# TheCacophonyProject/classifier-pipeline

Hardware: AMD Instinct MI355X
Metric: CPTV frames/s end-to-end (track+classify) at 160x120 (higher is better)
Workload: dtype u16/i32 track stage (f32 normalise, f64 gates); f32 crop/tile; f32 CNN (stride-1 3x3 convs of stages 2-4 (+ the stride-2 one): two fp16 planes per operand rounded to nearest (11 + 11 significand bits), power-of-two range scaling, 3 fp16 MFMAs per K step, device-side rerun in the exact split if an ac

## Files before the change

classifier-pipeline_amd/csrc/cpx_api.cpp:

```cpp
#include <hip/hip_runtime.h>

#include <algorithm>
#include <cmath>
#include <cstdio>
#include <cstdlib>
#include <cstring>
#include <new>
#include <string>
#include <vector>

#include "cpx_internal.h"

static_assert(sizeof(cpx_component) == 32, "cpx_component layout is part of the ABI");
static_assert(sizeof(cpx_frame_info) == 80, "cpx_frame_info layout is part of the ABI");
static_assert(sizeof(cpx_frame_meta) == 24, "cpx_frame_meta layout is part of the ABI");
static_assert(sizeof(cpx_config) == 48, "cpx_config layout is part of the ABI");
static_assert(sizeof(cpx_region_ref) == 24 && sizeof(cpx_track_limits) == 32 && sizeof(cpx_crop_req) == 32,
              "classification request layouts are part of the ABI");
static_assert(sizeof(cpx_filter_params) == 72 && sizeof(cpx_track_summary) == 120,
              "end-of-clip layouts are part of the ABI");
static_assert(sizeof(cpx_region) == 56, "cpx_region layout is part of the ABI");
static_assert(sizeof(cpx_track_record) == 32, "cpx_track_record layout is part of the ABI");
static_assert(sizeof(cpx_track_params) == 120, "cpx_track_params layout is part of the ABI");

namespace {

struct WsLayout {
  size_t bg, wsum, kcnt, filt, cstate, u8, carry, bgavg, big, total;
};

WsLayout ws_layout(const cpx_config& c, int B, bool need_filt_state) {
  const size_t P = (size_t)c.width * c.height;
  WsLayout l{};
  size_t off = 0;
  l.bg = off;
  off = align_up(off + (size_t)B * 2 * P * sizeof(uint16_t), 256);
  l.wsum = off;
  off = align_up(off + (size_t)B * P * sizeof(uint32_t), 256);
  l.kcnt = off;
  off = align_up(off + (size_t)B * P * sizeof(uint16_t), 256);
  l.filt = off;
  if (need_filt_state) off = align_up(off + (size_t)B * 2 * P * sizeof(float), 256);
  l.cstate = off;
  off = align_up(off + (size_t)B * sizeof(cpx::ClipState), 256);
  l.u8 = off;
  off = align_up(off + (size_t)B * 2 * P, 256);
  l.carry = off;
  off = align_up(off + (size_t)B * 2 * sizeof(cpx::FrameCarry), 256);
  l.bgavg = off;
  off = align_up(off + (size_t)B * sizeof(double), 256);
  l.big = off;
  if (c.max_components > cpx::track_lds_components())
    off = align_up(off + (size_t)B * 9 * c.max_components * sizeof(uint32_t), 256);
  l.total = off;
  return l;
}

struct Schedule {
  std::vector<int> clip_first, proc_off, proc_idx, proc_ffc, order;
  int total = 0, max_proc = 0;
};

int build_schedule(cpx_handle* h, const int32_t* clip_offsets, const cpx_frame_meta* meta, int B, Schedule* sc) {
  sc->total = clip_offsets[B];
  sc->clip_first.resize(B);
  sc->proc_off.assign(B + 1, 0);
  sc->proc_idx.reserve(sc->total);
  sc->proc_ffc.reserve(sc->total);
  for (int b = 0; b < B; ++b) {
    const int f0 = clip_offsets[b], f1 = clip_offsets[b + 1];
    if (f1 <= f0) return fail(h, CPX_ERR_INVALID, "empty clip in batch");
    sc->clip_first[b] = f0;
    for (int f = f0; f < f1; ++f) {
      if (meta[f].background_frame) continue;
      sc->proc_idx.push_back(f);
      int ffc = 0;
      if (meta[f].has_times) ffc = (meta[f].time_on_ms - meta[f].last_ffc_ms) < 9 ? 1 : 0;
      sc->proc_ffc.push_back(ffc);
    }
    sc->proc_off[b + 1] = (int)sc->proc_idx.size();
    const int np = sc->proc_off[b + 1] - sc->proc_off[b];
    if (np > h->cfg.max_frames) return fail(h, CPX_ERR_INVALID, "clip longer than max_frames");
    sc->max_proc = std::max(sc->max_proc, np);
  }
  sc->order.resize(B);
  for (int b = 0; b < B; ++b) sc->order[b] = b;
  std::stable_sort(sc->order.begin(), sc->order.end(), [&](int x, int y) {
    return sc->proc_off[x + 1] - sc->proc_off[x] > sc->proc_off[y + 1] - sc->proc_off[y];
  });
  return CPX_OK;
}

int upload_schedule(cpx_handle* h, const Schedule& sc, int B) {
  const int n = std::max((int)sc.proc_idx.size(), 1);
  const size_t ints = (size_t)B + (B + 1) + 2 * (size_t)n + (size_t)B;
  if (ints > h->sched_ints) {
    if (h->sched_dev) hipFree(h->sched_dev);
    h->sched_dev = nullptr;
    h->sched_ints = 0;
    hipError_t e = hipMalloc((void**)&h->sched_dev, ints * sizeof(int));
    if (e != hipSuccess) return fail(h, CPX_ERR_NOMEM, "schedule hipMalloc", e);
    h->sched_ints = ints;
  }
  std::vector<int> flat(ints, 0);
  std::copy(sc.clip_first.begin(), sc.clip_first.end(), flat.begin());
  std::copy(sc.proc_off.begin(), sc.proc_off.end(), flat.begin() + B);
  std::copy(sc.proc_idx.begin(), sc.proc_idx.end(), flat.begin() + B + (B + 1));
  std::copy(sc.proc_ffc.begin(), sc.proc_ffc.end(), flat.begin() + B + (B + 1) + n);
  std::copy(sc.order.begin(), sc.order.end(), flat.begin() + B + (B + 1) + 2 * (size_t)n);
  CPX_HIP(h, hipMemcpyAsync(h->sched_dev, flat.data(), ints * sizeof(int), hipMemcpyHostToDevice, h->stream));
  CPX_HIP(h, hipStreamSynchronize(h->stream));
  return CPX_OK;
}

}

extern "C" {

int cpx_abi_version(void) { return CPX_ABI_VERSION; }

int cpx_create(int device_id, const cpx_config* cfg, cpx_handle** out) {
  if (!cfg || !out) return CPX_ERR_INVALID;
  *out = nullptr;
  int ndev = 0;
  if (hipGetDeviceCount(&ndev) != hipSuccess || ndev <= 0) return CPX_ERR_NO_DEVICE;
  if (device_id < 0 || device_id >= ndev) return CPX_ERR_INVALID;
  const int W = cfg->width, H = cfg->height;
  if (W <= 0 || H <= 0 || (W % 8) != 0 || W >= 192 || W * H > cpx::track_max_pixels() || H < 5 || W < 8)
    return CPX_ERR_UNSUPPORTED;
  if (cfg->edge_pixels < 0 || 2 * cfg->edge_pixels >= std::min(W, H) || cfg->window < 1 ||
      cfg->max_components < 1 || cfg->max_frames < 1 || cfg->max_frames > 65534)
    return CPX_ERR_INVALID;
  cpx_handle* h = new (std::nothrow) cpx_handle();
  if (!h) return CPX_ERR_NOMEM;
  h->device = device_id;
  h->cfg = *cfg;
  if (hipSetDevice(device_id) != hipSuccess || hipStreamCreateWithFlags(&h->stream, hipStreamNonBlocking) != hipSuccess ||
      hipStreamCreateWithFlags(&h->stream2, hipStreamNonBlocking) != hipSuccess ||
      hipEventCreateWithFlags(&h->ev_median, hipEventDisableTiming) != hipSuccess ||
      hipEventCreate(&h->ev0) != hipSuccess || hipEventCreate(&h->ev1) != hipSuccess) {
    cpx_destroy(h);
    return CPX_ERR_HIP;
  }
  h->wtab_len = 65536;
  h->wtab_host.resize(h->wtab_len);
  std::vector<double>& wt = h->wtab_host;
  double w = 0.0;
  for (int k = 0; k < h->wtab_len; ++k) {
    wt[k] = w;
    w = w + cfg->weight_add;
  }
  if (cfg->denoise) {
    if (!cpx::nlm_supported(W, H)) {
      cpx_destroy(h);
      return CPX_ERR_UNSUPPORTED;
    }
    const int fixed_point_mult = (int)(2147483647LL / (21 * 21 * 255));
    std::vector<int> lut(64, 0);
    for (int a2 = 0; a2 < 64; ++a2) {
      const double wv = std::exp(-((double)a2 * (64.0 / 49.0)) / 9.0);
      const double wr = std::nearbyint((double)fixed_point_mult * wv);
      lut[a2] = (wr < 0.001 * fixed_point_mult) ? 0 : (int)wr;
    }
    if (lut[63] != 0 || hipMalloc((void**)&h->nlm_lut_dev, 64 * sizeof(int)) != hipSuccess ||
// ... 3 lines not shown
    }
  }
  std::vector<uint32_t> thr(h->wtab_len);
  for (int k = 0; k < h->wtab_len; ++k) {
    const double wk = wt[k], m = std::nearbyint(wk);
    const bool exact = (wk == m), near = !exact && std::fabs(wk - m) < 1e-6;
    double hi = near ? m + 1.0 : std::floor(wk) + 1.0;
    if (!(hi >= 0.0)) hi = 0.0;
    if (hi > 536870912.0) hi = 536870912.0;
    thr[k] = 2u * (uint32_t)hi - (near ? 1u : 0u);
  }
  if (hipMalloc((void**)&h->wthr_dev, thr.size() * sizeof(uint32_t)) != hipSuccess ||
      hipMemcpy(h->wthr_dev, thr.data(), thr.size() * sizeof(uint32_t), hipMemcpyHostToDevice) != hipSuccess) {
    cpx_destroy(h);
    return CPX_ERR_HIP;
  }
  if (hipMalloc(&h->wtab_dev, wt.size() * sizeof(double)) != hipSuccess ||
      hipMemcpy(h->wtab_dev, wt.data(), wt.size() * sizeof(double), hipMemcpyHostToDevice) != hipSuccess ||
      cpx::frame_kernel_attr_setup() != 0) {
    cpx_destroy(h);
    return CPX_ERR_HIP;
  }
  if (const char* env = std::getenv("CPX_TRACK_PACKED_STATE")) h->packed_state_ok = std::atoi(env) != 0;
  if (const char* env = std::getenv("CPX_CNN_FUSE_CONV1")) h->fuse_conv1 = std::atoi(env) != 0;
  if (const char* env = std::getenv("CPX_TRACK_PER_STEP")) h->track_per_step = std::atoi(env) != 0;
  if (const char* env = std::getenv("CPX_CNN_FUSE_SHORTCUT")) h->fuse_shortcut = std::atoi(env) != 0;
  if (const char* env = std::getenv("CPX_CNN_BLOCK_FUSION")) h->block_fusion = std::min(std::max(std::atoi(env), 0), 2);
  if (const char* env = std::getenv("CPX_CNN_MATH")) {
    if (!std::strcmp(env, "f32")) h->cnn_math = CPX_CNN_MATH_F32;
    else if (!std::strcmp(env, "bf16x3")) h->cnn_math = CPX_CNN_MATH_BF16X3;
    else if (!std::strcmp(env, "bf16x2")) h->cnn_math = CPX_CNN_MATH_BF16X2;
    else if (!std::strcmp(env, "fp16x2")) h->cnn_math = CPX_CNN_MATH_FP16X2;
  }
  *out = h;
  return CPX_OK;
}

void cpx_destroy(cpx_handle* h) {
  if (!h) return;
  hipSetDevice(h->device);
  if (h->stream) hipStreamSynchronize(h->stream);
  for (cpx_cnn* c : h->cnns) cnn_free(c);
  h->cnns.clear();
  for (cpx_mog2* m : h->mog2s) mog2_free(m);
  h->mog2s.clear();
  for (cpx_graph* g : h->graphs) graph_free(g);
  h->graphs.clear();
  if (h->graph_arena) hipFree(h->graph_arena);
  if (h->ws) hipFree(h->ws);
  if (h->wtab_dev) hipFree(h->wtab_dev);
  if (h->wthr_dev) hipFree(h->wthr_dev);
  if (h->nlm_lut_dev) hipFree(h->nlm_lut_dev);
  if (h->sched_dev) hipFree(h->sched_dev);
  if (h->ws_assoc) hipFree(h->ws_assoc);
  if (h->ir_scratch) hipFree(h->ir_scratch);
  if (h->bf3_scratch) hipFree(h->bf3_scratch);
  if (h->cnn_ovf) hipFree(h->cnn_ovf);
  if (h->cnn_arena) hipFree(h->cnn_arena);
  if (h->ir_bitmap) hipFree(h->ir_bitmap);
  for (auto& e : h->conv_events) {
    hipEventDestroy(e.e0);
    hipEventDestroy(e.e1);
  }
  if (h->stream2) {
    hipStreamSynchronize(h->stream2);
    hipStreamDestroy(h->stream2);
  }
  if (h->ev_median) hipEventDestroy(h->ev_median);
  if (h->ev0) hipEventDestroy(h->ev0);
  if (h->ev1) hipEventDestroy(h->ev1);
  if (h->stream) hipStreamDestroy(h->stream);
  delete h;
}

const char* cpx_last_error(const cpx_handle* h) { return h ? h->err.c_str() : "null handle"; }

void* cpx_stream(cpx_handle* h) { return h ? (void*)h->stream : nullptr; }

static int join_medians(cpx_handle* h) {
  if (h->medians_pending) {
    h->medians_pending = false;
    CPX_HIP(h, hipStreamWaitEvent(h->stream, h->ev_median, 0));
  }
  return CPX_OK;
}

int cpx_join_medians(cpx_handle* h) {
  if (!h) return CPX_ERR_INVALID;
  return join_medians(h);
}

int cpx_release_memory(cpx_handle* h) {
  if (!h) return CPX_ERR_INVALID;
  CPX_ENTER(h);
  if (int rc = join_medians(h)) return rc;
  CPX_HIP(h, hipStreamSynchronize(h->stream));
  CPX_HIP(h, hipStreamSynchronize(h->stream2));
  if (h->cnn_arena) hipFree(h->cnn_arena);
  h->cnn_arena = nullptr;
  h->cnn_arena_floats = 0;
  if (h->graph_arena) hipFree(h->graph_arena);
  h->graph_arena = nullptr;
  h->graph_arena_floats = 0;
  if (h->bf3_scratch) hipFree(h->bf3_scratch);
  h->bf3_scratch = nullptr;
  h->bf3_scratch_bytes = 0;
  if (h->ws) hipFree(h->ws);
  h->ws = nullptr;
  h->ws_bytes = 0;
  h->last_B = 0;
  h->state_packed = false;
  if (h->ws_assoc) hipFree(h->ws_assoc);
  h->ws_assoc = nullptr;
  h->ws_assoc_bytes = 0;
  if (h->ir_scratch) hipFree(h->ir_scratch);
  h->ir_scratch = nullptr;
  h->ir_scratch_bytes = 0;
  return CPX_OK;
}

int cpx_synchronize(cpx_handle* h) {
  if (!h) return CPX_ERR_INVALID;
  if (int rc = join_medians(h)) return rc;
  CPX_HIP(h, hipStreamSynchronize(h->stream));
  return CPX_OK;
}

size_t cpx_track_workspace_bytes(const cpx_handle* h, int B, int total_frames) {
  if (!h || B <= 0) return 0;
  (void)total_frames;
  return ws_layout(h->cfg, B, true).total;
}

static int unpack_state(cpx_handle* h) {
  if (h->state_packed && h->ws && h->last_B > 0) {
    const WsLayout lp = ws_layout(h->cfg, h->last_B, h->stream_filt_state);
    char* base = (char*)h->ws;
    cpx::launch_unpack_state((uint32_t*)(base + lp.wsum), (uint16_t*)(base + lp.kcnt),
                             (size_t)h->last_B * h->cfg.width * h->cfg.height, h->stream);
    CPX_HIP(h, hipGetLastError());
  }
  h->state_packed = false;
  return CPX_OK;
}

static int track_run(cpx_handle* h, const uint16_t* frames_dev, const int32_t* clip_offsets,
                     const cpx_frame_meta* meta, int B, int n_prev, cpx_component* comps_dev,
                     cpx_frame_info* info_dev, int32_t* labels_dev, float* filtered_dev,
                     float* background_dev, int flags) {
  CPX_ENTER(h);
  if (flags & ~(CPX_TRACK_KEEP_BACKGROUND | CPX_TRACK_FREEZE_ON_FFC | CPX_TRACK_FREEZE_BACKGROUND | CPX_TRACK_DEFER_MEDIANS))
    return fail(h, CPX_ERR_INVALID, "track: unknown flag");
  if (int jrc = join_medians(h)) return jrc;
  const bool defer_medians = (flags & CPX_TRACK_DEFER_MEDIANS) != 0;
  const cpx_config& c = h->cfg;
  Schedule sc;
  int rc = build_schedule(h, clip_offsets, meta, B, &sc);
  if (rc != CPX_OK) return rc;
  const int total = sc.total, max_proc = sc.max_proc;
  const bool resume = n_prev > 0;
  int t_begin = 0;
  if (resume)
    for (int f = 0; f < n_prev; ++f) t_begin += meta[f].background_frame ? 0 : 1;
  const bool need_filt = (filtered_dev == nullptr);
  const WsLayout l = ws_layout(c, B, need_filt);
  if (resume && (l.total > h->ws_bytes || need_filt != h->stream_filt_state))
    return fail(h, CPX_ERR_INVALID, "cpx_track_frame: the stream's workspace is gone (optional outputs changed?)");
  const bool keep = !resume && (flags & CPX_TRACK_KEEP_BACKGROUND);
  if (keep) {
    const bool have_prev = h->ws && h->last_B == B && need_filt == h->stream_filt_state && l.total <= h->ws_bytes;
    for (int b = 0; b < B && !have_prev; ++b)
      if (!h->staged_bg.count(b)) {
        h->staged_bg.clear();
        return fail(h, CPX_ERR_INVALID, "CPX_TRACK_KEEP_BACKGROUND: no background state for a clip (previous call had another batch size, and nothing staged; staged states dropped)");
      }
  }
  for (const auto& kv : h->staged_bg)
    if (kv.first >= B) {
      h->staged_bg.clear();
      return fail(h, CPX_ERR_INVALID, "cpx_set_background: staged clip index outside the batch (staged states dropped)");
    }
  if (resume || keep) {
    if (int urc = unpack_state(h)) return urc;
  }
  h->state_packed = false;
  h->stream_filt_state = need_filt;
  h->last_B = B;
  struct StateGuard {
    cpx_handle* h;
    bool armed = true;
    ~StateGuard() {
      if (armed) {
        h->last_B = 0;
        h->state_packed = false;
      }
    }
  } guard{h};
  if (l.total > h->ws_bytes) {
    if (h->ws) hipFree(h->ws);
    h->ws = nullptr;
    h->ws_bytes = 0;
    hipError_t e = hipMalloc(&h->ws, l.total);
    if (e != hipSuccess) return fail(h, CPX_ERR_NOMEM, "workspace hipMalloc", e);
    h->ws_bytes = l.total;
  }
  rc = upload_schedule(h, sc, B);
  if (rc != CPX_OK) return rc;
  const int nproc_total = (int)sc.proc_idx.size();

  cpx::TrackArgs a{};
  a.W = c.width;
  a.H = c.height;
  a.edge = c.edge_pixels;
  a.window = c.window;
  a.cap_out = c.max_components;
  a.flags = flags;
  a.background_thresh = c.background_thresh;
  a.weight_add = c.weight_add;
  a.frames = frames_dev;
  a.clip_first = h->sched_dev;
  a.proc_off = h->sched_dev + B;
  a.proc_idx = h->sched_dev + B + (B + 1);
  a.proc_ffc = h->sched_dev + B + (B + 1) + std::max(nproc_total, 1);
  a.order = h->sched_dev + B + (B + 1) + 2 * (size_t)std::max(nproc_total, 1);
  a.wtab = h->wtab_dev;
  a.wtab_len = h->wtab_len;
  a.wthr = h->wthr_dev;
  char* base = (char*)h->ws;
  a.bg = (uint16_t*)(base + l.bg);
  a.wsum = (uint32_t*)(base + l.wsum);
  a.kcnt = (uint16_t*)(base + l.kcnt);
  a.packed_state = (h->packed_state_ok && !resume && !keep && h->staged_bg.empty() && max_proc <= 1023 && c.window <= 64) ? 1 : 0;
  a.filt_state = need_filt ? (float*)(base + l.filt) : nullptr;
  a.cstate = (cpx::ClipState*)(base + l.cstate);
  a.u8_state = (unsigned char*)(base + l.u8);
  a.carry = (cpx::FrameCarry*)(base + l.carry);
  a.bgavg = (double*)(base + l.bgavg);
  a.big_stat = c.max_components > cpx::track_lds_components() ? (uint32_t*)(base + l.big) : nullptr;
  a.nlm_flip = c.denoise ? 1 : 0;
  a.nlm_lut = h->nlm_lut_dev;
  a.comps_out = comps_dev;
  a.info_out = info_dev;
  a.labels_out = labels_dev;
  a.filtered_out = filtered_dev;

  const int f_new = resume ? n_prev : 0;
  CPX_HIP(h, hipMemsetAsync(info_dev + f_new, 0xFF, (size_t)(total - f_new) * sizeof(cpx_frame_info), h->stream));
  if (!resume) cpx::launch_init(a, B, keep ? 1 : 0, h->stream);
  if (!h->staged_bg.empty()) {
    const size_t P = (size_t)c.width * c.height;
    for (const auto& kv : h->staged_bg) {
      const int b = kv.first;
      const auto& sb = kv.second;
      for (int slot = 0; slot < 2; ++slot)
        CPX_HIP(h, hipMemcpyAsync(a.bg + ((size_t)b * 2 + slot) * P, sb.bg.data(), P * sizeof(uint16_t),
                                  hipMemcpyHostToDevice, h->stream));
      CPX_HIP(h, hipMemcpyAsync(a.kcnt + (size_t)b * P, sb.kcnt.data(), P * sizeof(uint16_t), hipMemcpyHostToDevice,
                                h->stream));
      CPX_HIP(h, hipMemcpyAsync(&a.cstate[b].bg_average, &sb.average, sizeof(double), hipMemcpyHostToDevice, h->stream));
      CPX_HIP(h, hipMemcpyAsync(a.bgavg + b, &sb.average, sizeof(double), hipMemcpyHostToDevice, h->stream));
    }
// ... 117 lines not shown
}

int cpx_get_background(cpx_handle* h, int clip, float* background, double* weights, double* average) {
  if (!h) return CPX_ERR_INVALID;
  if (clip < 0 || clip >= h->last_B || !h->ws) return fail(h, CPX_ERR_INVALID, "cpx_get_background: no such clip in the last track call");
  CPX_ENTER(h);
  const cpx_config& c = h->cfg;
  const int W = c.width, H = c.height, e = c.edge_pixels;
  const size_t P = (size_t)W * H;
  const WsLayout l = ws_layout(c, h->last_B, h->stream_filt_state);
  char* base = (char*)h->ws;
  if (int urc = unpack_state(h)) return urc;
  CPX_HIP(h, hipStreamSynchronize(h->stream));
  cpx::ClipState st;
  CPX_HIP(h, hipMemcpy(&st, base + l.cstate + (size_t)clip * sizeof(cpx::ClipState), sizeof(st), hipMemcpyDeviceToHost));
  if (average) *average = st.bg_average;
  if (background) {
    std::vector<uint16_t> bg(P);
    CPX_HIP(h, hipMemcpy(bg.data(), base + l.bg + ((size_t)clip * 2 + (st.n_done & 1)) * P * sizeof(uint16_t),
                         P * sizeof(uint16_t), hipMemcpyDeviceToHost));
    for (int y = 0; y < H; ++y)
      for (int x = 0; x < W; ++x) {
        const int cy = std::min(std::max(y, e), H - 1 - e), cx = std::min(std::max(x, e), W - 1 - e);
        background[(size_t)y * W + x] = (float)bg[(size_t)cy * W + cx];
      }
  }
  if (weights) {
    std::vector<uint16_t> kc(P);
    CPX_HIP(h, hipMemcpy(kc.data(), base + l.kcnt + (size_t)clip * P * sizeof(uint16_t), P * sizeof(uint16_t),
                         hipMemcpyDeviceToHost));
    const std::vector<double>& wt = h->wtab_host;
    const int iw = W - 2 * e, ih = H - 2 * e;
    for (int y = 0; y < ih; ++y)
      for (int x = 0; x < iw; ++x) {
        const int k = kc[(size_t)(y + e) * W + (x + e)];
        weights[(size_t)y * iw + x] = k < h->wtab_len ? wt[k] : (double)k * c.weight_add;
      }
  }
  return CPX_OK;
}

static int assoc_run(cpx_handle* h, const cpx_track_params* params, const int32_t* clip_offsets,
                     const cpx_frame_meta* meta, int B, int n_prev, bool fresh, const cpx_component* comps_dev,
                     const cpx_frame_info* info_dev, cpx_region* pool_dev,
                     cpx_track_record* tracks_dev, int32_t* n_tracks_dev, int32_t* status_dev,
                     cpx_region* regions_dev, int32_t* region_counts_dev) {
  if (params->max_active_tracks < 1 || params->max_tracks < 1)
    return fail(h, CPX_ERR_INVALID, "association: capacities must be positive");
  CPX_ENTER(h);
  const bool resume = n_prev > 0 && !fresh;
  int t_begin = 0;
  if (n_prev > 0)
    for (int f = 0; f < n_prev; ++f) t_begin += meta[f].background_frame ? 0 : 1;
  Schedule sc;
  int rc = build_schedule(h, clip_offsets, meta, B, &sc);
  if (rc != CPX_OK) return rc;
  rc = upload_schedule(h, sc, B);
  if (rc != CPX_OK) return rc;
  const int n = std::max((int)sc.proc_idx.size(), 1);
  const int cap = h->cfg.max_components, ma = params->max_active_tracks;
  size_t off = 0;
  const size_t o_active = off;
  off = align_up(off + (size_t)B * ma * cpx::assoc_active_bytes(), 256);
  const size_t o_regs = off;
  off = align_up(off + (size_t)B * cap * sizeof(cpx_region), 256);
  const size_t o_scores = off;
  off = align_up(off + (size_t)B * cap * ma * cpx::assoc_score_bytes(), 256);
  const size_t o_used = off;
  off = align_up(off + (size_t)B * cap, 256);
  const size_t o_resume = off;
  off = align_up(off + (size_t)B * sizeof(cpx::AssocResume), 256);
  if (resume && off > h->ws_assoc_bytes)
    return fail(h, CPX_ERR_INVALID, "cpx_associate_frame: the stream's association state is gone");
  if (off > h->ws_assoc_bytes) {
    if (h->ws_assoc) hipFree(h->ws_assoc);
    h->ws_assoc = nullptr;
    h->ws_assoc_bytes = 0;
    hipError_t e = hipMalloc(&h->ws_assoc, off);
    if (e != hipSuccess) return fail(h, CPX_ERR_NOMEM, "association workspace hipMalloc", e);
    h->ws_assoc_bytes = off;
  }
  char* base = (char*)h->ws_assoc;
  cpx::AssocArgs a{};
  a.B = B;
  a.cap = cap;
  a.params = *params;
  a.clip_first = h->sched_dev;
  a.proc_off = h->sched_dev + B;
  a.proc_idx = h->sched_dev + B + (B + 1);
  a.proc_ffc = h->sched_dev + B + (B + 1) + n;
  a.comps = comps_dev;
  a.info = info_dev;
  a.pool = pool_dev;
  a.tracks = tracks_dev;
  a.n_tracks = n_tracks_dev;
  a.status = status_dev;
  a.regions_out = regions_dev;
  a.region_counts = region_counts_dev;
  a.active = (cpx::ActiveTrack*)(base + o_active);
  a.regs = (cpx_region*)(base + o_regs);
  a.scores = (cpx::ScoreRec*)(base + o_scores);
  a.used = (unsigned char*)(base + o_used);
  a.resume = (cpx::AssocResume*)(base + o_resume);
  a.t_begin = t_begin;
  a.fresh = resume ? 0 : 1;
  cpx::launch_assoc(a, h->stream);
  CPX_HIP(h, hipGetLastError());
  return CPX_OK;
}

int cpx_associate_batch(cpx_handle* h, const cpx_track_params* params, const int32_t* clip_offsets,
                        const cpx_frame_meta* meta, int B, const cpx_component* comps_dev,
// ... 51 lines not shown
                              const cpx_frame_info* info_dev, const cpx_region_ref* refs_dev,
                              const int32_t* track_offsets_dev, int n_tracks, cpx_track_limits* limits_dev, int flags) {
  if (!h) return CPX_ERR_INVALID;
  if (!frames_dev || !filtered_dev || !info_dev || !refs_dev || !track_offsets_dev || !limits_dev || n_tracks < 0 ||
      (flags & ~(CPX_LIMITS_POST_PROCESS | CPX_LIMITS_THERMAL_DIFF_NORM | CPX_LIMITS_NO_DIFF_NORM | CPX_LIMITS_ALWAYS_CLIP |
                 CPX_LIMITS_SWAP_CHANNELS | CPX_LIMITS_TF_SCALING)))
    return fail(h, CPX_ERR_INVALID, "cpx_track_limits_batch: bad argument");
  if (n_tracks == 0) return CPX_OK;
  CPX_ENTER(h);
  if (int jrc = join_medians(h)) return jrc;
  cpx::ClassifyArgs a = classify_args(h);
  a.limits_flags = flags;
  a.frames = frames_dev;
  a.filtered = filtered_dev;
  a.info = info_dev;
  a.refs = refs_dev;
  a.track_offsets = track_offsets_dev;
  a.limits = limits_dev;
  cpx::launch_limits(a, n_tracks, h->stream);
  CPX_HIP(h, hipGetLastError());
  return CPX_OK;
}

int cpx_crop_tile(cpx_handle* h, const uint16_t* frames_dev, const float* filtered_dev,
                  const cpx_frame_info* info_dev, const cpx_crop_req* reqs_dev, int n_reqs,
                  const cpx_track_limits* limits_dev, int frame_size, int square_width, float* out_dev) {
  if (!h) return CPX_ERR_INVALID;
  if (!frames_dev || !filtered_dev || !info_dev || !reqs_dev || !limits_dev || !out_dev || n_reqs < 0)
    return fail(h, CPX_ERR_INVALID, "cpx_crop_tile: null argument");
  if (frame_size < 1 || frame_size > 128 || square_width < 1 || square_width > 16)
    return fail(h, CPX_ERR_UNSUPPORTED, "cpx_crop_tile: frame_size must be 1..128, square_width 1..16");
  if (n_reqs == 0) return CPX_OK;
  CPX_ENTER(h);
  if (int jrc = join_medians(h)) return jrc;
  cpx::ClassifyArgs a = classify_args(h);
  a.frames = frames_dev;
  a.filtered = filtered_dev;
  a.info = info_dev;
  a.limits = const_cast<cpx_track_limits*>(limits_dev);
  a.reqs = reqs_dev;
  a.out = out_dev;
  a.frame_size = frame_size;
  a.square_width = square_width;
  cpx::launch_crop(a, n_reqs, h->stream);
  CPX_HIP(h, hipGetLastError());
  return CPX_OK;
}

static int final_common(cpx_handle* h, const cpx_filter_params* params, const int32_t* clip_offsets,
                        const cpx_frame_meta* meta, int B, cpx::FinalArgs* a) {
  if (params->max_active_tracks < 1 || params->max_tracks_per_clip < 1)
    return fail(h, CPX_ERR_INVALID, "filter params: capacities must be positive");
  CPX_ENTER(h);
  Schedule sc;
  int rc = build_schedule(h, clip_offsets, meta, B, &sc);
  if (rc != CPX_OK) return rc;
  rc = upload_schedule(h, sc, B);
  if (rc != CPX_OK) return rc;
  const int n = std::max((int)sc.proc_idx.size(), 1);
  a->B = B;
  a->params = *params;
  a->max_frames = h->cfg.max_frames;
  a->clip_first = h->sched_dev;
  a->proc_off = h->sched_dev + B;
  a->proc_idx = h->sched_dev + B + (B + 1);
  a->proc_ffc = h->sched_dev + B + (B + 1) + n;
  return CPX_OK;
}

static int final_scratch(cpx_handle* h, int B, cpx::FinalArgs* a) {
  const size_t need = (size_t)B * h->cfg.max_frames * (2 * sizeof(double) + sizeof(float)) + 512;
  if (need > h->ws_assoc_bytes) {
    CPX_HIP(h, hipStreamSynchronize(h->stream));
    if (h->ws_assoc) hipFree(h->ws_assoc);
    h->ws_assoc = nullptr;
    h->ws_assoc_bytes = 0;
    hipError_t e = hipMalloc(&h->ws_assoc, need);
    if (e != hipSuccess) return fail(h, CPX_ERR_NOMEM, "finalize workspace hipMalloc", e);
    h->ws_assoc_bytes = need;
  }
  a->scratch_d = (double*)h->ws_assoc;
  a->scratch_f = (float*)((char*)h->ws_assoc + align_up((size_t)B * h->cfg.max_frames * 2 * sizeof(double), 256));
  return CPX_OK;
}

int cpx_finalize_tracks(cpx_handle* h, const cpx_filter_params* params, const int32_t* clip_offsets,
                        const cpx_frame_meta* meta, int B, const cpx_region* pool_dev,
                        const cpx_track_record* tracks_dev, const int32_t* n_tracks_dev,
                        cpx_track_summary* summaries_dev, int32_t* counts_dev) {
  if (!h) return CPX_ERR_INVALID;
  if (!params || !clip_offsets || !meta || B <= 0 || !pool_dev || !tracks_dev || !n_tracks_dev || !summaries_dev ||
      !counts_dev)
    return fail(h, CPX_ERR_INVALID, "cpx_finalize_tracks: null argument");
  cpx::FinalArgs a{};
  int rc = final_common(h, params, clip_offsets, meta, B, &a);
  if (rc != CPX_OK) return rc;
  rc = final_scratch(h, B, &a);
  if (rc != CPX_OK) return rc;
  a.square_width = 5;
  a.pool = pool_dev;
  a.tracks = tracks_dev;
  a.n_tracks = n_tracks_dev;
  a.summaries = summaries_dev;
  a.counts = counts_dev;
  cpx::launch_finalize(a, h->stream);
  CPX_HIP(h, hipGetLastError());
  return CPX_OK;
}

int cpx_plan_segments(cpx_handle* h, const cpx_filter_params* params, const int32_t* clip_offsets,
                      const cpx_frame_meta* meta, int B, const cpx_region* pool_dev,
                      const cpx_track_summary* summaries_dev, const int32_t* n_tracks_dev,
// ... 201 lines not shown
```

classifier-pipeline_amd/csrc/cpx_internal.h:

```cpp
#pragma once
#include <hip/hip_runtime.h>

#include <map>
#include <string>
#include <vector>

#include "cpx.h"
#include "cpx_kernels.h"

struct cpx_cnn;
struct cpx_mog2;
struct cpx_graph;
void cnn_free(cpx_cnn* c);
void graph_free(cpx_graph* g);
void mog2_free(cpx_mog2* m);

struct cpx_handle {
  int device = 0;
  cpx_config cfg{};
  hipStream_t stream = nullptr;
  std::string err;
  void* ws = nullptr;
  size_t ws_bytes = 0;
  double* wtab_dev = nullptr;
  uint32_t* wthr_dev = nullptr;
  int wtab_len = 0;
  std::vector<double> wtab_host;
  int* nlm_lut_dev = nullptr;
  int* sched_dev = nullptr;
  size_t sched_ints = 0;
  struct ConvEv { int key; double flops; hipEvent_t e0, e1; };
  std::vector<ConvEv> conv_events;
  bool conv_timing = false;
  void* ws_assoc = nullptr;
  size_t ws_assoc_bytes = 0;
  hipEvent_t ev0 = nullptr, ev1 = nullptr;
  int last_launches = 0;
  bool timing_valid = false;
  hipStream_t stream2 = nullptr;
  bool state_packed = false;
  bool packed_state_ok = true;
  bool fuse_conv1 = true;
  bool medians_pending = false;
  hipEvent_t ev_median = nullptr;
  bool track_per_step = false;
  std::vector<struct cpx_cnn*> cnns;
  std::vector<struct cpx_mog2*> mog2s;
  std::vector<struct cpx_graph*> graphs;
  float* graph_arena = nullptr;
  size_t graph_arena_floats = 0;
  int stream_frames = -1;
  int stream_assoc_frames = -1;
  bool stream_filt_state = false;
  int last_B = 0;
  struct StagedBackground { std::vector<uint16_t> bg, kcnt; double average; };
  std::map<int, StagedBackground> staged_bg;
  int cnn_math = CPX_CNN_MATH_FP16X2;
  bool fuse_shortcut = true;
  void* bf3_scratch = nullptr;
  size_t bf3_scratch_bytes = 0;
  float* cnn_arena = nullptr;
  size_t cnn_arena_floats = 0;
  int* cnn_ovf = nullptr;
  int block_fusion = 2;
  unsigned char* ir_scratch = nullptr;
  size_t ir_scratch_bytes = 0;
  uint32_t* ir_bitmap = nullptr;
};

inline int fail(cpx_handle* h, int code, const char* what, hipError_t e = hipSuccess) {
  if (h) {
    h->err = what;
    if (e != hipSuccess) {
      h->err += ": ";
      h->err += hipGetErrorString(e);
    }
  }
  return code;
}

#define CPX_HIP(h, call)                                            \
  do {                                                              \
    hipError_t _e = (call);                                         \
// ... 11 lines not shown
```

classifier-pipeline_amd/csrc/cpx_kernels.h:

```cpp
#pragma once
#include <hip/hip_runtime.h>
#include <stddef.h>
#include <stdint.h>

#include "cpx.h"

#ifndef CPX_TRACK_THREADS
#define CPX_TRACK_THREADS 768
#endif
#ifndef CPX_TRACK_CHUNKS
#define CPX_TRACK_CHUNKS 7
#endif
#ifndef CPX_TRACK_LDS_COMPONENTS
#define CPX_TRACK_LDS_COMPONENTS 256
#endif
#ifndef CPX_TRACK_MIN_WAVES_PER_SIMD
#define CPX_TRACK_MIN_WAVES_PER_SIMD 6
#endif

namespace cpx {

typedef cpx_component Component;
typedef cpx_frame_info FrameInfo;

// ... 288 lines not shown
void launch_ir_frame_stats(const IrStatsArgs& a, hipStream_t s);
int ir_supported(int W, int H);
size_t ir_slot_bytes(int W, int H);

struct Mog2Args {
  size_t n;
  float alphaT, alpha1, prune;
  float var_threshold, background_ratio, var_threshold_gen, var_init, var_min, var_max;
  const unsigned char* frames;
  float* weight;
  float* var;
  float* mean;
  unsigned char* modes;
  unsigned char* mask;
};
void launch_mog2_apply(const Mog2Args& a, hipStream_t s);
void launch_mog2_background(const Mog2Args& a, unsigned char* out, hipStream_t s);

struct GraphView {
  float* p;
  int H, W, C, cstride;
  size_t sample_stride;
};
struct GraphOpArgs {
  int kind;
  int N;
  GraphView in0, in1, out;
  int kh, kw, stride_h, stride_w, pad_top, pad_left;
  int act;
  int n_map, map[4];
  float param;
  const float* weights;
  const float* scale;
  const float* shift;
};
void launch_graph_op(const GraphOpArgs& a, hipStream_t s);
constexpr int GRAPH_CONV_KC = 16;
constexpr int GRAPH_CONV_CO = 32;

inline bool cpx_dyn_lds_ready(const void* fn, bool* done, int bytes) {
  int dev = 0;
  if (hipGetDevice(&dev) != hipSuccess || dev < 0 || dev >= 64) return false;
  if (!done[dev]) {
    if (hipFuncSetAttribute(fn, hipFuncAttributeMaxDynamicSharedMemorySize, bytes) != hipSuccess) return false;
    done[dev] = true;
  }
  return true;
}

size_t track_lds_bytes(int W, int H);
int track_max_pixels();
int track_lds_components();
int frame_kernel_attr_setup();
void launch_init(const TrackArgs& a, int B, int keep, hipStream_t s);
void launch_unpack_state(uint32_t* wsum, uint16_t* kcnt, size_t n, hipStream_t s);
void launch_frame(const TrackArgs& a, int B, int t0, int t1, int mode, hipStream_t s);
void launch_nlm(const TrackArgs& a, int B, int t, hipStream_t s);
void launch_median(const TrackArgs& a, int B, int t0, int t1, hipStream_t s);
size_t nlm_lds_bytes(int W, int H);
int nlm_supported(int W, int H);
void launch_export_background(const TrackArgs& a, int B, float* out, hipStream_t s);

}
```

classifier-pipeline_amd/csrc/cpx_track.hip:

```cpp
#include <hip/hip_runtime.h>
#include <algorithm>
#include <cstdlib>
#include <type_traits>
#include <stdint.h>

#include "cpx_kernels.h"

namespace cpx {

namespace {

constexpr int NT = CPX_TRACK_THREADS;
constexpr int NWAVE = NT / 64;
constexpr int NCH = CPX_TRACK_CHUNKS;
constexpr int RW = 3;
constexpr int CAP = CPX_TRACK_LDS_COMPONENTS;
typedef unsigned long long u64;
typedef unsigned int u32;

__device__ __forceinline__ int clampi(int v, int lo, int hi) { return v < lo ? lo : (v > hi ? hi : v); }
template <typename T>
__device__ __forceinline__ T* at_off(T* base, unsigned bytes) {
  return reinterpret_cast<T*>(reinterpret_cast<char*>(base) + bytes);
}
// ... 1374 lines not shown
  }
}

namespace {
size_t nlm_lds_rows(int W, int rows, int bh) {
  const size_t ES = ((size_t)W + 2 * NLM_R + 8 + 7) & ~(size_t)7;
  const size_t HS = ((size_t)W + 24 + 7) & ~(size_t)7;
  const size_t nbuf = 2;
  return ((((size_t)rows + 2 * NLM_R) * ES + 32 + 15) & ~(size_t)15) + nbuf * ((size_t)rows + 16 + bh) * HS * 2 + NLM_LUT2 * NLM_LUT2 * 4 + 64;
}
template <int BH, int WC>
void launch_nlm_tw(const TrackArgs& a, int B, int t, hipStream_t s) {
  static bool lds_ready[64];
  (void)cpx_dyn_lds_ready(reinterpret_cast<const void*>(cpx_nlm_kernel<BH, WC>), lds_ready, 160 * 1024 - 2048);
  const int RB = BH * (NT_NLM / (a.W / 2));
  hipLaunchKernelGGL((cpx_nlm_kernel<BH, WC>), dim3(B, (a.H + RB - 1) / RB), dim3(NT_NLM),
                     nlm_lds_rows(a.W, RB < a.H ? RB : a.H, BH), s, a, t);
}
template <int BH>
void launch_nlm_t(const TrackArgs& a, int B, int t, hipStream_t s) {
  if (a.W == 160) launch_nlm_tw<BH, 160>(a, B, t, s);
  else launch_nlm_tw<BH, 0>(a, B, t, s);
}
}

size_t nlm_lds_bytes(int W, int H) {
  const int rb = 10 * (NT_NLM / (W / 2));
  return nlm_lds_rows(W, rb < H ? rb : H, 10);
}
int nlm_supported(int W, int H) {
  const int nsub = NT_NLM / (W / 2);
  return nsub >= 1 && (W % 8) == 0 && W >= 8 && H >= 1 && nlm_lds_bytes(W, H) <= 160 * 1024 - 2048;
}
void launch_nlm(const TrackArgs& a, int B, int t, hipStream_t s) {
  const int nsub = NT_NLM / (a.W / 2);
  const int want = (B >= 384) ? 1 : (512 + B - 1) / B;
  const int rows = (a.H + want - 1) / want;
  if (rows > 5 * nsub) launch_nlm_t<10>(a, B, t, s);
  else if (rows > 2 * nsub) launch_nlm_t<5>(a, B, t, s);
  else if (rows > nsub) launch_nlm_t<2>(a, B, t, s);
  else launch_nlm_t<1>(a, B, t, s);
}

__global__ __launch_bounds__(256) void cpx_export_background_kernel(TrackArgs a, float* out) {
  const int b = blockIdx.x;
  const int W = a.W, H = a.H, P = W * H, e = a.edge;
  const uint16_t* bg = a.bg + ((size_t)b * 2 + (a.cstate[b].n_done & 1)) * P;
  for (int p = threadIdx.x; p < P; p += blockDim.x) {
    int y = p / W, x = p - y * W;
    out[(size_t)b * P + p] = (float)bg[clampi(y, e, H - 1 - e) * W + clampi(x, e, W - 1 - e)];
  }
}

size_t track_lds_bytes(int W, int H) { return wtab_lds_offset(W, H) + (size_t)WTAB_LDS * sizeof(double) + (size_t)WTHR_LDS * sizeof(u32); }

void launch_init(const TrackArgs& a, int B, int keep, hipStream_t s) {
  hipLaunchKernelGGL(cpx_init_kernel, dim3(B), dim3(256), 0, s, a, keep);
}
void launch_frame(const TrackArgs& a, int B, int t0, int t1, int mode, hipStream_t s) {
  if (a.packed_state) hipLaunchKernelGGL(cpx_frame_kernel<true>, dim3(B), dim3(NT), track_lds_bytes(a.W, a.H), s, a, t0, t1, mode);
  else hipLaunchKernelGGL(cpx_frame_kernel<false>, dim3(B), dim3(NT), track_lds_bytes(a.W, a.H), s, a, t0, t1, mode);
}
__global__ __launch_bounds__(256) void cpx_unpack_state_kernel(uint32_t* wsum, uint16_t* kcnt, size_t n) {
  for (size_t i = (size_t)blockIdx.x * blockDim.x + threadIdx.x; i < n; i += (size_t)gridDim.x * blockDim.x) {
    const uint32_t v = wsum[i];
    kcnt[i] = (uint16_t)(v >> 22);
    wsum[i] = v & 0x3FFFFFu;
  }
}
void launch_unpack_state(uint32_t* wsum, uint16_t* kcnt, size_t n, hipStream_t s) {
  if (n == 0) return;
  const unsigned blocks = (unsigned)std::min<size_t>((n + 255) / 256, 65535u * 16u);
  hipLaunchKernelGGL(cpx_unpack_state_kernel, dim3(blocks), dim3(256), 0, s, wsum, kcnt, n);
}
void launch_median(const TrackArgs& a, int B, int t0, int t1, hipStream_t s) {
  if (t1 <= t0) return;
  hipLaunchKernelGGL(cpx_median_kernel, dim3((unsigned)(t1 - t0) * (unsigned)B), dim3(NT_MED), 0, s, a, t0, t1 - t0);
}
void launch_export_background(const TrackArgs& a, int B, float* out, hipStream_t s) {
  hipLaunchKernelGGL(cpx_export_background_kernel, dim3(B), dim3(256), 0, s, a, out);
}
int track_max_pixels() { return 4 * NCH * NT; }
int track_lds_components() { return CAP; }
int frame_kernel_attr_setup() {
  const int r0 = (int)hipFuncSetAttribute(reinterpret_cast<const void*>(cpx_frame_kernel<false>), hipFuncAttributeMaxDynamicSharedMemorySize, 160 * 1024 - 2048);
  const int r1 = (int)hipFuncSetAttribute(reinterpret_cast<const void*>(cpx_frame_kernel<true>), hipFuncAttributeMaxDynamicSharedMemorySize, 160 * 1024 - 2048);
  return r0 != 0 ? r0 : r1;
}

}
```

Measured before the change: 3.091 million.

## Cache frame schedule across calls and build index lists on device

Replaces the per-call host-built schedule and its synchronous upload with a cached version. Schedule data is now reused when clip offsets and per-frame codes are unchanged, copied from pinned memory asynchronously with an event instead of a stream sync, and expanded on the GPU by a ballot/popcount scan kernel. The aim is to remove host vector building and a blocking synchronize from every tracking, association and filter call. In exchange it adds cached state and a pending-copy event that must be handled correctly, plus an extra small kernel launch whenever the schedule changes.

```diff
diff --git a/classifier-pipeline_amd/csrc/cpx_api.cpp b/classifier-pipeline_amd/csrc/cpx_api.cpp
--- a/classifier-pipeline_amd/csrc/cpx_api.cpp
+++ b/classifier-pipeline_amd/csrc/cpx_api.cpp
@@ -56,44 +56,22 @@
   return l;
 }
 
-struct Schedule {
-  std::vector<int> clip_first, proc_off, proc_idx, proc_ffc, order;
-  int total = 0, max_proc = 0;
-};
-
-int build_schedule(cpx_handle* h, const int32_t* clip_offsets, const cpx_frame_meta* meta, int B, Schedule* sc) {
-  sc->total = clip_offsets[B];
-  sc->clip_first.resize(B);
-  sc->proc_off.assign(B + 1, 0);
-  sc->proc_idx.reserve(sc->total);
-  sc->proc_ffc.reserve(sc->total);
-  for (int b = 0; b < B; ++b) {
-    const int f0 = clip_offsets[b], f1 = clip_offsets[b + 1];
-    if (f1 <= f0) return fail(h, CPX_ERR_INVALID, "empty clip in batch");
-    sc->clip_first[b] = f0;
-    for (int f = f0; f < f1; ++f) {
-      if (meta[f].background_frame) continue;
-      sc->proc_idx.push_back(f);
-      int ffc = 0;
-      if (meta[f].has_times) ffc = (meta[f].time_on_ms - meta[f].last_ffc_ms) < 9 ? 1 : 0;
-      sc->proc_ffc.push_back(ffc);
-    }
-    sc->proc_off[b + 1] = (int)sc->proc_idx.size();
-    const int np = sc->proc_off[b + 1] - sc->proc_off[b];
-    if (np > h->cfg.max_frames) return fail(h, CPX_ERR_INVALID, "clip longer than max_frames");
-    sc->max_proc = std::max(sc->max_proc, np);
-  }
-  sc->order.resize(B);
-  for (int b = 0; b < B; ++b) sc->order[b] = b;
-  std::stable_sort(sc->order.begin(), sc->order.end(), [&](int x, int y) {
-    return sc->proc_off[x + 1] - sc->proc_off[x] > sc->proc_off[y + 1] - sc->proc_off[y];
-  });
-  return CPX_OK;
-}
-
-int upload_schedule(cpx_handle* h, const Schedule& sc, int B) {
-  const int n = std::max((int)sc.proc_idx.size(), 1);
-  const size_t ints = (size_t)B + (B + 1) + 2 * (size_t)n + (size_t)B;
+int join_medians(cpx_handle* h) {
+  if (h->medians_pending) {
+    h->medians_pending = false;
+    CPX_HIP(h, hipStreamWaitEvent(h->stream, h->ev_median, 0));
+  }
+  return CPX_OK;
+}
+
+inline unsigned char frame_code(const cpx_frame_meta& m) {
+  const unsigned proc = m.background_frame == 0;
+  const unsigned ffc = (unsigned)(m.has_times != 0) &
+                       (unsigned)((int64_t)((uint64_t)m.time_on_ms - (uint64_t)m.last_ffc_ms) < 9);
+  return (unsigned char)(proc | ((proc & ffc) << 1));
+}
+
+int schedule_buffers(cpx_handle* h, size_t ints, size_t pin_bytes) {
   if (ints > h->sched_ints) {
     if (h->sched_dev) hipFree(h->sched_dev);
     h->sched_dev = nullptr;
@@ -102,14 +80,86 @@
     if (e != hipSuccess) return fail(h, CPX_ERR_NOMEM, "schedule hipMalloc", e);
     h->sched_ints = ints;
   }
-  std::vector<int> flat(ints, 0);
-  std::copy(sc.clip_first.begin(), sc.clip_first.end(), flat.begin());
-  std::copy(sc.proc_off.begin(), sc.proc_off.end(), flat.begin() + B);
-  std::copy(sc.proc_idx.begin(), sc.proc_idx.end(), flat.begin() + B + (B + 1));
-  std::copy(sc.proc_ffc.begin(), sc.proc_ffc.end(), flat.begin() + B + (B + 1) + n);
-  std::copy(sc.order.begin(), sc.order.end(), flat.begin() + B + (B + 1) + 2 * (size_t)n);
-  CPX_HIP(h, hipMemcpyAsync(h->sched_dev, flat.data(), ints * sizeof(int), hipMemcpyHostToDevice, h->stream));
-  CPX_HIP(h, hipStreamSynchronize(h->stream));
+  if (h->sched_copy_pending) {
+    CPX_HIP(h, hipEventSynchronize(h->ev_sched));
+    h->sched_copy_pending = false;
+  }
+  if (pin_bytes > h->sched_pin_bytes) {
+    if (h->sched_pin) hipHostFree(h->sched_pin);
+    h->sched_pin = nullptr;
+    h->sched_pin_bytes = 0;
+    hipError_t e = hipHostMalloc(&h->sched_pin, pin_bytes, hipHostMallocDefault);
+    if (e != hipSuccess) return fail(h, CPX_ERR_NOMEM, "schedule hipHostMalloc", e);
+    h->sched_pin_bytes = pin_bytes;
+  }
+  return CPX_OK;
+}
+
+int ensure_schedule(cpx_handle* h, const int32_t* clip_offsets, const cpx_frame_meta* meta, int B) {
+  if (clip_offsets[0] < 0) return fail(h, CPX_ERR_INVALID, "negative clip offset");
+  bool same = h->sched_valid && h->sched_B == B &&
+              std::memcmp(h->sched_offsets.data(), clip_offsets, ((size_t)B + 1) * sizeof(int32_t)) == 0;
+  h->sched_valid = false;
+  int nb = 0;
+  while (nb < B && clip_offsets[nb + 1] > clip_offsets[nb]) ++nb;
+  const int total = clip_offsets[nb];
+  h->sched_codes.resize((size_t)total);
+  h->sched_counts.resize((size_t)B);
+  unsigned char* codes = h->sched_codes.data();
+  unsigned diff = 0;
+  int max_proc = 0;
+  long long nproc = 0;
+  for (int b = 0; b < nb; ++b) {
+    const int f0 = clip_offsets[b], f1 = clip_offsets[b + 1];
+    int np = 0;
+    for (int f = f0; f < f1; ++f) {
+      const unsigned char c = frame_code(meta[f]);
+      diff |= (unsigned)(c ^ codes[f]);
+      codes[f] = c;
+      np += c & 1;
+    }
+    if (np > h->cfg.max_frames) return fail(h, CPX_ERR_INVALID, "clip longer than max_frames");
+    h->sched_counts[b] = np;
+    max_proc = std::max(max_proc, np);
+    nproc += np;
+  }
+  if (nb < B) return fail(h, CPX_ERR_INVALID, "empty clip in batch");
+  h->sched_max_proc = max_proc;
+  h->sched_nproc = (int)nproc;
+  if (same && diff == 0) {
+    h->sched_valid = true;
+    return CPX_OK;
+  }
+  h->sched_B = B;
+  h->sched_offsets.assign(clip_offsets, clip_offsets + B + 1);
+  if (int rc = join_medians(h)) return rc;
+  const size_t n = (size_t)std::max(h->sched_nproc, 1);
+  const size_t head = (size_t)B + (B + 1), tail_at = head + 2 * n;
+  const size_t ints = tail_at + (size_t)B + ((size_t)total + 3) / 4;
+  const size_t pin_bytes = (head + (size_t)B) * sizeof(int) + (size_t)total;
+  if (int rc = schedule_buffers(h, ints, pin_bytes)) return rc;
+  int* st = (int*)h->sched_pin;
+  int* st_off = st + B;
+  int* st_order = st + head;
+  st_off[0] = 0;
+  for (int b = 0; b < B; ++b) {
+    st[b] = clip_offsets[b];
+    st_off[b + 1] = st_off[b] + h->sched_counts[b];
+    st_order[b] = b;
+  }
+  const int* counts = h->sched_counts.data();
+  std::stable_sort(st_order, st_order + B, [counts](int x, int y) { return counts[x] > counts[y]; });
+  std::memcpy(st_order + B, codes, (size_t)total);
+  if (!h->ev_sched) CPX_HIP(h, hipEventCreateWithFlags(&h->ev_sched, hipEventDisableTiming));
+  int* dev = h->sched_dev;
+  h->sched_copy_pending = true;
+  CPX_HIP(h, hipMemcpyAsync(dev, st, head * sizeof(int), hipMemcpyHostToDevice, h->stream));
+  CPX_HIP(h, hipMemcpyAsync(dev + tail_at, st_order, (size_t)B * sizeof(int) + (size_t)total, hipMemcpyHostToDevice, h->stream));
+  CPX_HIP(h, hipEventRecord(h->ev_sched, h->stream));
+  cpx::launch_schedule_scan((const unsigned char*)(dev + tail_at + B), dev, dev + B, B, total, dev + head, dev + head + n,
+                            h->stream);
+  CPX_HIP(h, hipGetLastError());
+  h->sched_valid = true;
   return CPX_OK;
 }
 
@@ -219,6 +269,8 @@
   if (h->wthr_dev) hipFree(h->wthr_dev);
   if (h->nlm_lut_dev) hipFree(h->nlm_lut_dev);
   if (h->sched_dev) hipFree(h->sched_dev);
+  if (h->sched_pin) hipHostFree(h->sched_pin);
+  if (h->ev_sched) hipEventDestroy(h->ev_sched);
   if (h->ws_assoc) hipFree(h->ws_assoc);
   if (h->ir_scratch) hipFree(h->ir_scratch);
   if (h->bf3_scratch) hipFree(h->bf3_scratch);
@@ -243,14 +295,6 @@
 const char* cpx_last_error(const cpx_handle* h) { return h ? h->err.c_str() : "null handle"; }
 
 void* cpx_stream(cpx_handle* h) { return h ? (void*)h->stream : nullptr; }
-
-static int join_medians(cpx_handle* h) {
-  if (h->medians_pending) {
-    h->medians_pending = false;
-    CPX_HIP(h, hipStreamWaitEvent(h->stream, h->ev_median, 0));
-  }
-  return CPX_OK;
-}
 
 int cpx_join_medians(cpx_handle* h) {
   if (!h) return CPX_ERR_INVALID;
@@ -321,10 +365,9 @@
   if (int jrc = join_medians(h)) return jrc;
   const bool defer_medians = (flags & CPX_TRACK_DEFER_MEDIANS) != 0;
   const cpx_config& c = h->cfg;
-  Schedule sc;
-  int rc = build_schedule(h, clip_offsets, meta, B, &sc);
+  int rc = ensure_schedule(h, clip_offsets, meta, B);
   if (rc != CPX_OK) return rc;
-  const int total = sc.total, max_proc = sc.max_proc;
+  const int total = clip_offsets[B], max_proc = h->sched_max_proc;
   const bool resume = n_prev > 0;
   int t_begin = 0;
   if (resume)
@@ -371,9 +414,7 @@
     if (e != hipSuccess) return fail(h, CPX_ERR_NOMEM, "workspace hipMalloc", e);
     h->ws_bytes = l.total;
   }
-  rc = upload_schedule(h, sc, B);
-  if (rc != CPX_OK) return rc;
-  const int nproc_total = (int)sc.proc_idx.size();
+  const int nproc_total = h->sched_nproc;
 
   cpx::TrackArgs a{};
   a.W = c.width;
@@ -597,12 +638,9 @@
   int t_begin = 0;
   if (n_prev > 0)
     for (int f = 0; f < n_prev; ++f) t_begin += meta[f].background_frame ? 0 : 1;
-  Schedule sc;
-  int rc = build_schedule(h, clip_offsets, meta, B, &sc);
+  int rc = ensure_schedule(h, clip_offsets, meta, B);
   if (rc != CPX_OK) return rc;
-  rc = upload_schedule(h, sc, B);
-  if (rc != CPX_OK) return rc;
-  const int n = std::max((int)sc.proc_idx.size(), 1);
+  const int n = std::max(h->sched_nproc, 1);
   const int cap = h->cfg.max_components, ma = params->max_active_tracks;
   size_t off = 0;
   const size_t o_active = off;
@@ -760,12 +798,9 @@
   if (params->max_active_tracks < 1 || params->max_tracks_per_clip < 1)
     return fail(h, CPX_ERR_INVALID, "filter params: capacities must be positive");
   CPX_ENTER(h);
-  Schedule sc;
-  int rc = build_schedule(h, clip_offsets, meta, B, &sc);
+  int rc = ensure_schedule(h, clip_offsets, meta, B);
   if (rc != CPX_OK) return rc;
-  rc = upload_schedule(h, sc, B);
-  if (rc != CPX_OK) return rc;
-  const int n = std::max((int)sc.proc_idx.size(), 1);
+  const int n = std::max(h->sched_nproc, 1);
   a->B = B;
   a->params = *params;
   a->max_frames = h->cfg.max_frames;
diff --git a/classifier-pipeline_amd/csrc/cpx_internal.h b/classifier-pipeline_amd/csrc/cpx_internal.h
--- a/classifier-pipeline_amd/csrc/cpx_internal.h
+++ b/classifier-pipeline_amd/csrc/cpx_internal.h
@@ -29,6 +29,16 @@
   int* nlm_lut_dev = nullptr;
   int* sched_dev = nullptr;
   size_t sched_ints = 0;
+  bool sched_valid = false;
+  int sched_B = 0;
+  std::vector<int32_t> sched_offsets;
+  std::vector<unsigned char> sched_codes;
+  std::vector<int> sched_counts;
+  int sched_max_proc = 0, sched_nproc = 0;
+  void* sched_pin = nullptr;
+  size_t sched_pin_bytes = 0;
+  hipEvent_t ev_sched = nullptr;
+  bool sched_copy_pending = false;
   struct ConvEv { int key; double flops; hipEvent_t e0, e1; };
   std::vector<ConvEv> conv_events;
   bool conv_timing = false;
diff --git a/classifier-pipeline_amd/csrc/cpx_kernels.h b/classifier-pipeline_amd/csrc/cpx_kernels.h
--- a/classifier-pipeline_amd/csrc/cpx_kernels.h
+++ b/classifier-pipeline_amd/csrc/cpx_kernels.h
@@ -364,6 +364,8 @@
 int track_max_pixels();
 int track_lds_components();
 int frame_kernel_attr_setup();
+void launch_schedule_scan(const unsigned char* codes, const int* clip_first, const int* proc_off, int B, int total,
+                          int* proc_idx, int* proc_ffc, hipStream_t s);
 void launch_init(const TrackArgs& a, int B, int keep, hipStream_t s);
 void launch_unpack_state(uint32_t* wsum, uint16_t* kcnt, size_t n, hipStream_t s);
 void launch_frame(const TrackArgs& a, int B, int t0, int t1, int mode, hipStream_t s);
diff --git a/classifier-pipeline_amd/csrc/cpx_track.hip b/classifier-pipeline_amd/csrc/cpx_track.hip
--- a/classifier-pipeline_amd/csrc/cpx_track.hip
+++ b/classifier-pipeline_amd/csrc/cpx_track.hip
@@ -1450,7 +1450,33 @@
   }
 }
 
-size_t track_lds_bytes(int W, int H) { return wtab_lds_offset(W, H) + (size_t)WTAB_LDS * sizeof(double) + (size_t)WTHR_LDS * sizeof(u32); }
+__global__ __launch_bounds__(64) void cpx_schedule_scan_kernel(const unsigned char* __restrict__ codes,
+                                                                const int* __restrict__ clip_first,
+                                                                const int* __restrict__ proc_off, int B, int total,
+                                                                int* __restrict__ proc_idx, int* __restrict__ proc_ffc) {
+  const int b = blockIdx.x, lane = threadIdx.x;
+  const int f0 = clip_first[b], f1 = b + 1 < B ? clip_first[b + 1] : total;
+  const int end = proc_off[b + 1];
+  int pos = proc_off[b];
+  for (int g = f0; g < f1; g += 64) {
+    const int f = g + lane;
+    const int code = f < f1 ? codes[f] : 0;
+    const unsigned long long m = __ballot(code & 1);
+    const int at = pos + __popcll(m & ((1ull << lane) - 1ull));
+    if ((code & 1) && at < end) {
+      proc_idx[at] = f;
+      proc_ffc[at] = (code >> 1) & 1;
+    }
+    pos += __popcll(m);
+  }
+}
+void launch_schedule_scan(const unsigned char* codes, const int* clip_first, const int* proc_off, int B, int total,
+                          int* proc_idx, int* proc_ffc, hipStream_t s) {
+  hipLaunchKernelGGL(cpx_schedule_scan_kernel, dim3(B), dim3(64), 0, s, codes, clip_first, proc_off, B, total, proc_idx,
+                     proc_ffc);
+}
+
+size_t track_lds_bytes(int W, int H) { return wtab_lds_offset(W, H)+ (size_t)WTAB_LDS * sizeof(double) + (size_t)WTHR_LDS * sizeof(u32); }
 
 void launch_init(const TrackArgs& a, int B, int keep, hipStream_t s) {
   hipLaunchKernelGGL(cpx_init_kernel, dim3(B), dim3(256), 0, s, a, keep);
diff --git a/scratch/step_gaps.py b/scratch/step_gaps.py
--- /dev/null
+++ b/scratch/step_gaps.py
@@ -0,0 +1,41 @@
+import csv, sys
+rows = list(csv.DictReader(open(sys.argv[1])))
+iv = sorted((int(r["Start_Timestamp"]), int(r["End_Timestamp"]), r["Kernel_Name"]) for r in rows)
+frames = [i for i, x in enumerate(iv) if "cpx_frame_kernel" in x[2]]
+i0, i1 = frames[-2], frames[-1]
+t0 = iv[i0][0]
+def short(n):
+    n = n.replace("cpx::(anonymous namespace)::", "").replace("cpx::", "").replace("void ", "")
+    return n.split("(")[0][:60]
+prev_end = max(e for _, e, _ in iv[:i0])
+print("previous step's last kernel end -> frame kernel start: %.2f ms" % ((t0 - prev_end) / 1e6))
+cur_end = t0
+run = None
+idle = busy = 0
+out = []
+marks = {}
+for s, e, n in iv[i0:i1]:
+    gap = s - cur_end
+    if gap >= 100000:
+        if run: out.append(run); run = None
+        out.append(("   idle", gap, s - gap - t0, 0))
+    if gap > 0: idle += gap
+    for key in ("cpx_assoc_kernel", "cpx_finalize_kernel", "cpx_plan_kernel"):
+        if key in n: marks[key] = max(gap, 0)
+    if run and run[0] == short(n):
+        run = (run[0], run[1] + (e - s), run[2], run[3] + 1)
+    else:
+        if run: out.append(run)
+        run = (short(n), e - s, s - t0, 1)
+    busy += max(0, e - max(s, cur_end))
+    cur_end = max(cur_end, e)
+if run: out.append(run)
+for name, ns, at, cnt in out:
+    print("+%8.2f ms  %8.2f ms  x%-4d %s" % (at / 1e6, ns / 1e6, cnt, name))
+tail = iv[i1][0] - cur_end
+print("last kernel end -> next frame kernel start: %.2f ms" % (tail / 1e6))
+for key, gap in marks.items():
+    print("idle in front of %s: %.2f ms" % (key, gap / 1e6))
+copies = [x for x in iv[i0:i1] if "copyBuffer" in x[2] and x[1] - x[0] >= 20000]
+print("staged copies of at least 0.02 ms in the step: %d" % len(copies))
+print("step (frame kernel to frame kernel) %.2f ms, busy %.2f ms, idle %.2f ms" % ((iv[i1][0] - t0) / 1e6, busy / 1e6, (idle + tail) / 1e6))
```

Result: no change. 3.111 million, median of 5 (+0.6%).
